# mclarsen/cuZFP

Measured on AMD Instinct MI355X. Metric: GB/s input encoded+decoded (device-resident), 3D f32 fixed-rate; % HBM peak, higher is better.
Workload: dtype f32; 1 GPU; 3d_float32_256^3_rate8; maxbits=512, parallelism=z-slab x1, stream_bytes_per_gpu=16777216

## Files before the change

cuzfp_amd/build.py:

```python
from __future__ import annotations

import os
import subprocess
import sys
from concurrent.futures import ThreadPoolExecutor

HERE = os.path.dirname(os.path.abspath(__file__))
ROOT = os.path.dirname(HERE)
CSRC = os.path.join(HERE, "csrc")
LIB = os.path.join(HERE, "lib")
BIN = os.path.join(HERE, "bin")
CLI = os.path.join(HERE, "cli")
OBJ = os.path.join(ROOT, "build", "obj")
INC = os.path.join(ROOT, "include")

ARCH = os.environ.get("CUZFP_OFFLOAD_ARCH", "gfx950")
HIPCC = os.environ.get("HIPCC", "/opt/rocm/bin/hipcc")
CXXFLAGS = ["-O3", "-std=c++17", "-fPIC", f"--offload-arch={ARCH}", f"-I{INC}",
            "-Wall", "-Wno-unused-function", "-Wno-pass-failed"]

KERNEL_UNITS = ["inst_f32", "inst_f64", "inst_i32", "inst_i64",
                "region_f32", "region_f64", "region_i32", "region_i64",
                "update_f32", "update_f64", "update_i32", "update_i64", "truncate",
                "variable_f32", "variable_f64", "region_variable_f32", "region_variable_f64", "truncate_variable",
                "region_variable_coarse_f32", "region_variable_coarse_f64",
                "region_variable_update_f32", "region_variable_update_f64",
                "capi"]
HEADERS = ["zfp_block.hpp", "kernels.hpp", "launch.hpp", "region.hpp", "region_kernels.hpp",
           "region_update_kernels.hpp", "rerate.hpp", "variable_kernels.hpp", "variable_index.hpp",
           "region_variable_kernels.hpp", "rerate_variable.hpp", "source_window.hpp", "variable_coarse.hpp",
           "region_variable_coarse_kernels.hpp", "region_variable_update_kernels.hpp"]


def _newer(target: str, deps: list[str]) -> bool:
    if not os.path.exists(target):
        return True
    t = os.path.getmtime(target)
    return any(os.path.getmtime(d) > t for d in deps)


def _run(cmd: list[str]) -> None:
    r = subprocess.run(cmd, capture_output=True, text=True)
    if r.returncode != 0:
        sys.stderr.write(r.stdout + r.stderr)
        raise RuntimeError("build failed: " + " ".join(cmd))


def build(verbose: bool = False, jobs: int | None = None) -> dict:
    os.makedirs(LIB, exist_ok=True)
    os.makedirs(OBJ, exist_ok=True)
    hdrs = [os.path.join(CSRC, h) for h in HEADERS] + [os.path.join(INC, "cuzfp_hip.h")]
    jobs_list = []
    objs = []
    for u in KERNEL_UNITS:
        src = os.path.join(CSRC, u + ".hip")
        obj = os.path.join(OBJ, u + ".o")
        objs.append(obj)
        if _newer(obj, [src] + hdrs):
            jobs_list.append([HIPCC, *CXXFLAGS, "-c", src, "-o", obj])
    with ThreadPoolExecutor(max_workers=jobs or min(8, os.cpu_count() or 4)) as ex:
        for cmd in jobs_list:
            if verbose:
                print(" ".join(cmd))
        list(ex.map(_run, jobs_list))
    hip_so = os.path.join(LIB, "libcuzfp_hip.so")
    if jobs_list or _newer(hip_so, objs):
        _run([HIPCC, f"--offload-arch={ARCH}", "-shared", "-fPIC", "-o", hip_so, *objs])
    cpp_src = os.path.join(CSRC, "cuZFP.cpp")
    cpp_so = os.path.join(LIB, "libcuZFP.so")
    if _newer(cpp_so, [cpp_src, hip_so, os.path.join(INC, "cuZFP.h"),
                       os.path.join(INC, "zfp_structs.h")]):
        _run([HIPCC, "-O2", "-std=c++17", "-fPIC", "-shared", f"-I{INC}", "-o", cpp_so, cpp_src,
              f"-L{LIB}", "-lcuzfp_hip", "-Wl,-rpath,$ORIGIN"])
    os.makedirs(BIN, exist_ok=True)
    cli = os.path.join(BIN, "cuda_zfp")
    if _newer(cli, [os.path.join(CLI, "cuda_zfp.cpp"), cpp_so, os.path.join(INC, "cuZFP.h"),
                    os.path.join(INC, "zfp_structs.h")]):
        _run(["g++", "-O2", "-std=c++17", "-Wall", "-Wno-unused-function", f"-I{INC}", "-o", cli,
              os.path.join(CLI, "cuda_zfp.cpp"), f"-L{LIB}", "-lcuZFP", "-Wl,-rpath,$ORIGIN/../lib"])
    gen = os.path.join(BIN, "data_gen")
    if _newer(gen, [os.path.join(CLI, "data_gen.cpp")]):
        _run(["g++", "-O2", "-std=c++17", "-Wall", "-o", gen, os.path.join(CLI, "data_gen.cpp")])
    return {"hip": hip_so, "cpp": cpp_so, "cli": cli, "data_gen": gen}


if __name__ == "__main__":
    print(build(verbose=True))
```

cuzfp_amd/csrc/capi.hip:

```cpp
#include <hip/hip_runtime.h>
#include <math.h>

#include <algorithm>
#include <cstring>
#include <mutex>
#include <chrono>
#include <vector>

#include "launch.hpp"
#include "rerate_variable.hpp"
#include "variable_index.hpp"

namespace cuzfp {

thread_local int t_last_hip = hipSuccess;

static unsigned min_bits(int type) { return type == CUZFP_TYPE_FLOAT ? 9 : type == CUZFP_TYPE_DOUBLE ? 12 : 1; }

static int make_problem(int type, unsigned nx, unsigned ny, unsigned nz, long long sx,
                        long long sy, long long sz, unsigned maxbits, Problem* pr) {
  if (type < CUZFP_TYPE_INT32 || type > CUZFP_TYPE_DOUBLE) return CUZFP_ERROR_UNSUPPORTED_TYPE;
  if (!nx || (nz && !ny)) return CUZFP_ERROR_INVALID_ARGUMENT;
  const unsigned dims = nz ? 3 : ny ? 2 : 1;
  const unsigned ebits = min_bits(type);
  if (maxbits < ebits || maxbits > CUZFP_MAX_BITS) return CUZFP_ERROR_INVALID_ARGUMENT;
  Geometry& g = pr->g;
  g.nx = nx;
  g.ny = dims > 1 ? ny : 1;
  g.nz = dims > 2 ? nz : 1;
  g.bx = (g.nx + 3) / 4;
  g.by = (g.ny + 3) / 4;
  const uint64_t nb = (uint64_t)g.bx * g.by * ((g.nz + 3) / 4);
  if (nb >= (1ull << 32) - kLanes) return CUZFP_ERROR_INVALID_ARGUMENT;
  g.nblocks = (uint32_t)nb;
  set_divisor(g.bx, g.dbx_m, g.dbx_s);
  set_divisor(g.bx * g.by, g.dpl_m, g.dpl_s);
  g.divmagic = nb < (1ull << 31) ? 1u : 0u;
  g.maxbits = maxbits;
  g.wave0 = 0;
  g.vec_io = 0;
  g.row_stage = 0;
  g.sx = sx ? sx : 1;
  g.sy = sy ? sy : (long long)g.nx;
  g.sz = sz ? sz : (long long)g.nx * g.ny;
  pr->type = type;
  pr->dims = dims;
  pr->fast_ok = (type == CUZFP_TYPE_FLOAT || type == CUZFP_TYPE_DOUBLE) && g.sx == 1 &&
                g.sy == (long long)g.nx && g.sz == (long long)g.nx * g.ny && g.nx % 4 == 0 &&
                (dims < 2 || g.ny % 4 == 0) && (dims < 3 || g.nz % 4 == 0);
  return CUZFP_SUCCESS;
}

static int launch_encode(const Problem& p, const void* data, uint64_t* stream, uint32_t wave0,
                         uint32_t nwaves, hipStream_t st) {
  if (!nwaves) return CUZFP_SUCCESS;
  const bool fast = p.fast_ok && ((uintptr_t)data & 15) == 0;
  switch (p.type) {
    case CUZFP_TYPE_INT32: return launch_encode_type<int32_t>(p, data, false, stream, wave0, nwaves, st);
    case CUZFP_TYPE_INT64: return launch_encode_type<int64_t>(p, data, false, stream, wave0, nwaves, st);
    case CUZFP_TYPE_FLOAT: return launch_encode_type<float>(p, data, fast, stream, wave0, nwaves, st);
    default: return launch_encode_type<double>(p, data, fast, stream, wave0, nwaves, st);
  }
}

static int launch_decode(const Problem& p, const uint64_t* stream, void* data, uint32_t wave0,
                         uint32_t nwaves, hipStream_t st) {
  if (!nwaves) return CUZFP_SUCCESS;
  const bool fast = p.fast_ok && ((uintptr_t)data & 15) == 0;
  switch (p.type) {
    case CUZFP_TYPE_INT32: return launch_decode_type<int32_t>(p, stream, false, data, wave0, nwaves, st);
    case CUZFP_TYPE_INT64: return launch_decode_type<int64_t>(p, stream, false, data, wave0, nwaves, st);
    case CUZFP_TYPE_FLOAT: return launch_decode_type<float>(p, stream, fast, data, wave0, nwaves, st);
    default: return launch_decode_type<double>(p, stream, fast, data, wave0, nwaves, st);
  }
}

static size_t stream_bytes_of(const Geometry& g) {
  return (((size_t)g.nblocks * g.maxbits + 63) / 64) * 8;
}

static uint32_t waves_of(const Geometry& g) { return (g.nblocks + kLanes - 1) / kLanes; }


typedef uint32_t u32x4 __attribute__((ext_vector_type(4)));

__global__ __launch_bounds__(256) void copy16_nt(const u32x4* __restrict__ src, u32x4* __restrict__ dst,
                                                 size_t n16) {
  const size_t stride = (size_t)gridDim.x * blockDim.x;
  for (size_t i = (size_t)blockIdx.x * blockDim.x + threadIdx.x; i < n16; i += stride)
    __builtin_nontemporal_store(__builtin_nontemporal_load(src + i), dst + i);
}


constexpr size_t kChunkBytes = 64u << 20, kStagedChunkBytes = 8u << 20;

static size_t chunk_bytes(bool staged) {
  const char* e = getenv("CUZFP_HOST_CHUNK_BYTES");
  if (e && *e) {
    const long long v = atoll(e);
    if (v > 0) return (size_t)v;
  }
  return staged ? kStagedChunkBytes : kChunkBytes;
}

static bool host_ordered() {
  const char* e = getenv("CUZFP_HOST_ORDERED");
  return !(e && *e == '0');
}

static int host_zero_copy() {
  const char* e = getenv("CUZFP_HOST_ZEROCOPY");
  return (e && *e) ? atoi(e) : 1;
}

static char* mapped_view(const void* p, size_t bytes) {
  hipPointerAttribute_t a;
  void* d = nullptr;
  hipDeviceptr_t base = nullptr;
  size_t size = 0;
  const bool ok = hipPointerGetAttributes(&a, p) == hipSuccess && a.type == hipMemoryTypeHost &&
                  hipHostGetDevicePointer(&d, const_cast<void*>(p), 0) == hipSuccess && d &&
                  hipMemGetAddressRange(&base, &size, (hipDeviceptr_t)d) == hipSuccess && base &&
                  (char*)d >= (char*)base && (size_t)((char*)d - (char*)base) + bytes <= size;
  (void)hipGetLastError();
// ... 1016 lines not shown
```

cuzfp_amd/csrc/kernels.hpp:

```cpp
#pragma once
#include <hip/hip_runtime.h>
#include <stdlib.h>

#include <atomic>
#include <type_traits>

#if defined(CUZFP_PROBE) && CUZFP_PROBE == 9
#define CUZFP_STAMP_WAVES 65536
__device__ uint64_t g_stamps[CUZFP_STAMP_WAVES * 10];
__device__ __forceinline__ uint32_t stamp_wave() { return blockIdx.x * (blockDim.x >> 6) + (threadIdx.x >> 6); }
#define ZFP_STAMP(i)                                                              \
  do {                                                                            \
    if ((threadIdx.x & 63) == 0 && stamp_wave() < CUZFP_STAMP_WAVES)              \
      g_stamps[stamp_wave() * 10 + 1 + (i)] = __builtin_amdgcn_s_memtime();      \
  } while (0)
__device__ __forceinline__ void stamp_hwid() {
  uint32_t hw, xcc;
  asm volatile("s_getreg_b32 %0, hwreg(HW_REG_HW_ID)" : "=s"(hw));
  asm volatile("s_getreg_b32 %0, hwreg(HW_REG_XCC_ID)" : "=s"(xcc));
  if ((threadIdx.x & 63) == 0 && stamp_wave() < CUZFP_STAMP_WAVES)
    g_stamps[stamp_wave() * 10] = (uint64_t)hw | ((uint64_t)xcc << 32);
}
__device__ __forceinline__ void stamp_real(int slot) {
  if ((threadIdx.x & 63) == 0 && stamp_wave() < CUZFP_STAMP_WAVES)
    g_stamps[stamp_wave() * 10 + slot] = __builtin_amdgcn_s_memrealtime();
}
#define ZFP_STAMP_REAL(slot) stamp_real(slot)
#define ZFP_STAMP_HWID() stamp_hwid()
#else
#define ZFP_STAMP_HWID()
#define ZFP_STAMP_REAL(slot)
#endif

#include "zfp_block.hpp"
#include "launch.hpp"

namespace cuzfp {

__device__ const ChunkLut g_chunk_lut = make_chunk_lut();
constexpr size_t kChunkLutBytes = sizeof(ChunkLut);
template <int DIMS>
constexpr size_t chunk_lut_bytes() { return DIMS == 1 ? kLutPairs * 4 : kChunkLutBytes; }
__device__ const SpreadTab g_spread_tab = make_spread_tab();
__device__ const Pair1dLut g_pair1d_lut = make_pair1d_lut();
__device__ const Plane1dDecLut g_plane1d_lut = make_plane1d_dec_lut();
constexpr size_t kSpreadTabBytes = sizeof(SpreadTab);
typedef __attribute__((address_space(3))) const uint32_t lds_spread;
typedef lds_spread* P1dPtr;

__device__ __forceinline__ void udivmod_uniform(uint32_t n, uint32_t d, uint32_t& q, uint32_t& r) {
  if (__builtin_expect((d & (d - 1)) == 0, 1)) {
    const uint32_t sh = (uint32_t)__builtin_ctz(d);
    q = n >> sh;
    r = n & (d - 1);
  } else {
    q = n / d;
    r = n % d;
  }
}


constexpr uint32_t kSlackWords = 6;
template <bool PRIO = true>
struct LdsOrWriter {
  static constexpr bool kPrio = PRIO;
  static constexpr bool kZeroInline = true;
  uint64_t* p;
  lds_spread* lut;
  uint32_t pos, lim;
  P1dPtr p1d;
  uint64_t fit_lim;
  __device__ __forceinline__ uint32_t pair1d(uint32_t o) const { return *(P1dPtr)((uintptr_t)p1d + o); }
  __device__ __forceinline__ bool full() const { return pos >= lim; }
  __device__ __forceinline__ void put(uint64_t v, unsigned n) {
    const uint32_t w = pos >> 6;
    uint64_t* q = p + w * 64;
    const uint64_t lo = v << (pos & 63u);
    const uint64_t hi = (v >> 1) >> ((pos ^ 63u) & 63u);
    atomicOr((unsigned long long*)&q[0], (unsigned long long)lo);
    atomicOr((unsigned long long*)&q[64], (unsigned long long)hi);
    pos += n;
  }
  __device__ __forceinline__ uint32_t sp0(uint32_t o) const { return *(lds_spread*)((uintptr_t)lut + o); }
  __device__ __forceinline__ uint32_t sp1(uint32_t o) const { return *(lds_spread*)((uintptr_t)(lut + 256) + o); }
  __device__ __forceinline__ uint32_t spread(uint32_t b) const { return lut[256 + b] >> 1; }
  __device__ __forceinline__ void zero_bit() { pos++; }
  __device__ __forceinline__ void lds_wait() const { __builtin_amdgcn_s_waitcnt(0xc07f); }
  __device__ __forceinline__ void finish() {}
  __device__ __forceinline__ void settle() { pos = pos < lim ? pos : lim; }
  __device__ __forceinline__ void mark_full(bool z) { pos = z ? lim : pos; }
};

template <bool PRIO = true>
struct LdsBitWriter {
  static constexpr bool kPrio = PRIO;
  uint64_t* lds;
  lds_spread* lut;
  uint32_t pos, end, cnt;
  uint64_t acc;
  P1dPtr p1d;
  uint64_t fit_lim;
  __device__ __forceinline__ uint32_t pair1d(uint32_t o) const { return *(P1dPtr)((uintptr_t)p1d + o); }
  __device__ __forceinline__ uint32_t sp0(uint32_t o) const { return *(lds_spread*)((uintptr_t)lut + o); }
  __device__ __forceinline__ uint32_t sp1(uint32_t o) const { return *(lds_spread*)((uintptr_t)(lut + 256) + o); }
  __device__ __forceinline__ uint32_t spread(uint32_t b) const { return lut[256 + b] >> 1; }
  __device__ __forceinline__ bool full() const { return pos + cnt >= end; }
  __device__ __forceinline__ void emit(uint64_t v) {
    if (pos >= end) return;
    const uint32_t room = end - pos;
    if (room < 64) v &= lowmask(room);
    const uint32_t w = pos >> 6, sh = pos & 63;
    atomicOr((unsigned long long*)&lds[w], (unsigned long long)(v << sh));
    if (sh) atomicOr((unsigned long long*)&lds[w + 1], (unsigned long long)(v >> (64 - sh)));
    pos += 64;
  }
  __device__ __forceinline__ void put(uint64_t v, unsigned n) {
    acc |= v << cnt;
    const unsigned c = cnt + n;
// ... 331 lines not shown
template <int DIMS>
__device__ __forceinline__ BlockPos block_pos(const Geometry& g, uint32_t b) {
  BlockPos p;
  if constexpr (DIMS == 1) {
    p.ix = b; p.iy = 0; p.iz = 0;
  } else if constexpr (DIMS == 2) {
    p.iy = g.divmagic ? div_magic(b, g.dbx_m, g.dbx_s) : b / g.bx;
    p.ix = b - p.iy * g.bx; p.iz = 0;
  } else {
    const uint32_t plane = g.bx * g.by;
    p.iz = g.divmagic ? div_magic(b, g.dpl_m, g.dpl_s) : b / plane;
    const uint32_t r = b - p.iz * plane;
    p.iy = g.divmagic ? div_magic(r, g.dbx_m, g.dbx_s) : r / g.bx;
    p.ix = r - p.iy * g.bx;
  }
  return p;
}

template <typename Scalar, int DIMS, bool FAST>
__device__ __forceinline__ void gather(const Scalar* __restrict__ data, const Geometry& g,
                                       BlockPos bp, Scalar* f) {
  constexpr int NY = DIMS > 1 ? 4 : 1, NZ = DIMS > 2 ? 4 : 1;
  if constexpr (FAST) {
    const Scalar* p = data + ((size_t)(4 * bp.iz) * g.ny + 4 * bp.iy) * g.nx + 4 * bp.ix;
#pragma unroll
    for (int z = 0; z < NZ; z++)
#pragma unroll
      for (int y = 0; y < NY; y++)
        load_row(p + ((size_t)z * g.ny + y) * g.nx, f + 16 * z + 4 * y);
  } else {
    const int wx = (int)min(4u, g.nx - 4 * bp.ix);
    const int wy = (int)min(4u, g.ny - 4 * bp.iy);
    const int wz = (int)min(4u, g.nz - 4 * bp.iz);
    const Scalar* p = data + (int64_t)(4 * bp.ix) * g.sx + (int64_t)(4 * bp.iy) * g.sy +
                      (int64_t)(4 * bp.iz) * g.sz;
#pragma unroll
    for (int z = 0; z < NZ; z++)
#pragma unroll
      for (int y = 0; y < NY; y++)
#pragma unroll
        for (int x = 0; x < 4; x++)
          f[16 * z + 4 * y + x] = p[(int64_t)pad_src(x, wx) * g.sx + (int64_t)pad_src(y, wy) * g.sy +
                                    (int64_t)pad_src(z, wz) * g.sz];
  }
}

template <typename Scalar, int DIMS, bool FAST>
__device__ __forceinline__ void scatter(Scalar* __restrict__ data, const Geometry& g, BlockPos bp,
                                        const Scalar* f) {
  constexpr int NY = DIMS > 1 ? 4 : 1, NZ = DIMS > 2 ? 4 : 1;
  if constexpr (FAST) {
    Scalar* p = data + ((size_t)(4 * bp.iz) * g.ny + 4 * bp.iy) * g.nx + 4 * bp.ix;
#pragma unroll
    for (int z = 0; z < NZ; z++)
#pragma unroll
      for (int y = 0; y < NY; y++)
        store_row(p + ((size_t)z * g.ny + y) * g.nx, f + 16 * z + 4 * y);
  } else {
    const int wx = (int)min(4u, g.nx - 4 * bp.ix);
    const int wy = (int)min(4u, g.ny - 4 * bp.iy);
    const int wz = (int)min(4u, g.nz - 4 * bp.iz);
    Scalar* p = data + (int64_t)(4 * bp.ix) * g.sx + (int64_t)(4 * bp.iy) * g.sy +
                (int64_t)(4 * bp.iz) * g.sz;
#pragma unroll
    for (int z = 0; z < NZ; z++)
#pragma unroll
      for (int y = 0; y < NY; y++)
#pragma unroll
        for (int x = 0; x < 4; x++)
          if (x < wx && y < wy && z < wz)
            p[(int64_t)x * g.sx + (int64_t)y * g.sy + (int64_t)z * g.sz] = f[16 * z + 4 * y + x];
  }
}


constexpr int kWavesPerGroup = 4;
#ifndef CUZFP_ENC_WPG
#define CUZFP_ENC_WPG 4
#endif
#ifndef CUZFP_DEC_WPG
#define CUZFP_DEC_WPG 4
#endif
constexpr int kEncWaves = CUZFP_ENC_WPG, kDecWaves = CUZFP_DEC_WPG;
#ifndef CUZFP_REG_WAVES_1D
#define CUZFP_REG_WAVES_1D 16
#endif
constexpr int kRegWaves1d = CUZFP_REG_WAVES_1D;
#ifndef CUZFP_REG_WAVES_2D
#define CUZFP_REG_WAVES_2D 4
#endif
constexpr int kRegWaves2d = CUZFP_REG_WAVES_2D;
#ifndef CUZFP_REG_DEC_BATCH_1D
#define CUZFP_REG_DEC_BATCH_1D 4
#endif
#ifndef CUZFP_REG_ENC_BATCH_1D
#define CUZFP_REG_ENC_BATCH_1D 2
#endif
#ifndef CUZFP_REG_BATCH_WAVES_1D
#define CUZFP_REG_BATCH_WAVES_1D 8
#endif
#ifndef CUZFP_REG_BATCH_MIN_WAVES
#define CUZFP_REG_BATCH_MIN_WAVES 32768
#endif
constexpr int kRegDecBatch1d = CUZFP_REG_DEC_BATCH_1D, kRegEncBatch1d = CUZFP_REG_ENC_BATCH_1D;
constexpr int kRegBatchWaves1d = CUZFP_REG_BATCH_WAVES_1D;
constexpr uint32_t kRegBatchMinWaves = CUZFP_REG_BATCH_MIN_WAVES;
#ifndef CUZFP_REG_BATCH_PRIO
#define CUZFP_REG_BATCH_PRIO 0
#endif

__device__ __forceinline__ uint32_t wave_in_group() {
  return __builtin_amdgcn_readfirstlane(threadIdx.x >> 6);
}

__device__ __forceinline__ void wave_lds_sync() {
  asm volatile("s_waitcnt lgkmcnt(0)" ::: "memory");
  __builtin_amdgcn_wave_barrier();
}

template <int ROWS>
__device__ __forceinline__ void scatter_f64_staged(double* __restrict__ data, const Geometry& g, BlockPos bp,
                                                   const double* f, bool coded, uint64_t* wave_lds,
                                                   uint32_t lane) {
  static_assert(16 % ROWS == 0, "rows a pass");
  uint4* stage = (uint4*)wave_lds;
  double* base = data + ((size_t)(4 * bp.iz) * g.ny + 4 * bp.iy) * g.nx + 4 * (bp.ix - lane);
#pragma unroll
  for (int r0 = 0; r0 < 16; r0 += ROWS) {
    if (coded) {
#pragma unroll
      for (int j = 0; j < ROWS; j++) {
        uint4 a, b;
        __builtin_memcpy(&a, f + 4 * (r0 + j), 16);
        __builtin_memcpy(&b, f + 4 * (r0 + j) + 2, 16);
        stage[j * 128 + 2 * lane] = a;
        stage[j * 128 + 2 * lane + 1] = b;
      }
    } else {
#pragma unroll
      for (int j = 0; j < ROWS; j++) {
        stage[j * 128 + 2 * lane] = uint4{0, 0, 0, 0};
        stage[j * 128 + 2 * lane + 1] = uint4{0, 0, 0, 0};
      }
    }
    wave_lds_sync();
#pragma unroll
    for (int j = 0; j < ROWS; j++) {
      const int r = r0 + j, z = r >> 2, y = r & 3;
      double* row = base + ((size_t)z * g.ny + y) * g.nx;
      st16<true>(row + 2 * lane, stage[j * 128 + lane]);
      st16<true>(row + 128 + 2 * lane, stage[j * 128 + 64 + lane]);
    }
    if (r0 + ROWS < 16) wave_lds_sync();
  }
}

#ifndef CUZFP_F64_ENC_WAVES
#define CUZFP_F64_ENC_WAVES 2
#endif
#ifndef CUZFP_F64_DEC_WAVES
#define CUZFP_F64_DEC_WAVES 2
#endif
#ifndef CUZFP_F32_DEC_WAVES
#define CUZFP_F32_DEC_WAVES 4
#endif
#ifndef CUZFP_F32_ENC_WAVES
// ... 82 lines not shown
    if (g.wave0 + (bid + 1) * (blockDim.x >> 6) <= g.wave_end) {
      asm volatile("s_waitcnt vmcnt(0)" ::: "memory");
      __syncthreads();
    }
    wave_lds_sync();
    LdsOrWriter<PRIO> wr{mine, lut, 0, 64 * W, p1d, uniform_const64(0x7fffu)};
    encode_block<Scalar, DIMS>(f, g.maxbits, wr);
  } else if (b < g.nblocks) {
    {
      wave_lds_sync();
      LdsBitWriter<PRIO> wr{lds, lut, lane * g.maxbits, (lane + 1) * g.maxbits, 0, 0, p1d, uniform_const64(0x7fffu)};
      encode_block<Scalar, DIMS>(f, g.maxbits, wr);
    }
  }
  if constexpr (PRIO) __builtin_amdgcn_s_setprio(3);
  wave_lds_sync();
  const uint32_t nb = min((uint32_t)kLanes, g.nblocks - wave * kLanes);
  const uint32_t nwords = (nb * g.maxbits + 63) >> 6;
  uint64_t* out = stream + (size_t)wave * g.maxbits;
  if constexpr (ALIGNED) {
    if (nb == kLanes && g.vec_io && !(W & 1)) {
      uint32_t s, j, ds, dj;
      udivmod_uniform(2 * lane, W, s, j);
      udivmod_uniform(128u, W, ds, dj);
      for (uint32_t k = 2 * lane; k < kLanes * W; k += 128) {
        uint4 v;
        const uint64_t a0 = lds[j * 64 + s], a1 = lds[(j + 1) * 64 + s];
        __builtin_memcpy(&v.x, &a0, 8);
        __builtin_memcpy(&v.z, &a1, 8);
        st16<true>(&out[k], v);
        j += dj;
        s += ds;
        if (j >= W) { j -= W; s++; }
      }
      ZFP_STAMP(6);
      ZFP_STAMP_REAL(9);
      return;
    }
  }
  if constexpr (ALIGNED) {
    if (b < g.nblocks) {
      const uint64_t* mine = lds + lane;
      uint64_t* dst = out + (size_t)lane * W;
      if (g.vec_io && !(W & 1)) {
        for (uint32_t j = 0; j < W; j += 2) {
          uint4 v;
          const uint64_t a0 = mine[j * 64], a1 = mine[(j + 1) * 64];
          __builtin_memcpy(&v.x, &a0, 8);
          __builtin_memcpy(&v.z, &a1, 8);
          st16<kNtStream>(&dst[j], v);
        }
      } else {
        for (uint32_t j = 0; j < W; j++) dst[j] = mine[j * 64];
      }
    }
  } else if (g.vec_io) {
    const uint32_t npairs = nwords >> 1;
    for (uint32_t j = lane; j < npairs; j += kLanes)
      ((uint4*)out)[j] = ((const uint4*)lds)[j];
    if ((nwords & 1) && lane == 0) out[nwords - 1] = lds[nwords - 1];
  } else {
    for (uint32_t j = lane; j < nwords; j += kLanes) out[j] = lds[j];
  }
  ZFP_STAMP(6);
  ZFP_STAMP_REAL(9);
}

template <typename Scalar, int DIMS, bool FAST, bool ALIGNED, bool PRIO = true, int REG = 0, int WPG = kEncWaves>
__global__ __launch_bounds__(kLanes * WPG, (occupancy<Scalar, DIMS, true>::value)) void zfp_encode(const Scalar* __restrict__ data,
                                                                      Geometry g,
                                                                      uint64_t* __restrict__ stream) {
  __shared__ __attribute__((aligned(16))) uint32_t stab[512];
  __shared__ __attribute__((aligned(16))) uint32_t ptab[DIMS == 1 ? 1024 : 4];
  zfp_encode_body<Scalar, DIMS, FAST, ALIGNED, PRIO, REG, WPG>(data, g, stream, blockIdx.x, stab, ptab);
}

template <typename Scalar, int DIMS, bool FAST, bool PRIO = true, int REG = 0, int WPG = kDecWaves>
__device__ __forceinline__ void zfp_decode_body(const uint64_t* __restrict__ stream, const Geometry& g,
                                                Scalar* __restrict__ data, uint32_t bid,
                                                uint32_t* ctab, uint16_t* dtab) {
  extern __shared__ __attribute__((aligned(16))) uint64_t lds_all[];
  constexpr int N = 1 << (2 * DIMS);
  const uint32_t wig = wave_in_group();
  const uint32_t wave = g.wave0 + bid * (blockDim.x >> 6) + wig;
  const uint32_t lane = threadIdx.x & 63;
  const uint32_t b = wave * kLanes + lane;
  const bool live = wave < g.wave_end && b < g.nblocks;
  uint64_t* lds = lds_all + (size_t)wig * g.lds_words;
  uint32_t* lut = ctab;
  auto copy_dtab = [&]() {
    if constexpr (DIMS == 1)
      for (uint32_t i = threadIdx.x; i < sizeof(Plane1dDecLut) / 16; i += blockDim.x)
        ((uint4*)dtab)[i] = ((const uint4*)g_plane1d_lut.e)[i];
  };
  constexpr uint32_t kLutEnd = DIMS == 1 ? kLutPairs * 4 / 16 : sizeof(ChunkLut) / 16;
  const uint32_t* seg = (const uint32_t*)(stream + (size_t)wave * g.maxbits);
  uint32_t* L = (uint32_t*)lds + lane;
  uint64_t blk = 0;
  if constexpr (REG == 32) {
    if (live) blk = seg[lane];
    for (uint32_t i = threadIdx.x; i < kLutEnd; i += blockDim.x)
      ((uint4*)lut)[i] = ((const uint4*)g_chunk_lut.e)[i];
    copy_dtab();
  } else if constexpr (REG) {
    if (live) {
      const uint32_t nb = min((uint32_t)kLanes, g.nblocks - wave * kLanes);
      const uint32_t lim = ((nb * g.maxbits + 63) >> 6) * 2;
      const uint32_t s0 = lane * g.maxbits, d0 = s0 >> 5;
      const uint32_t a0 = seg[d0];
      const uint32_t a1 = d0 + 1 < lim ? seg[d0 + 1] : 0u;
      const uint32_t a2 = d0 + 2 < lim ? seg[d0 + 2] : 0u;
      blk = ((uint64_t)__builtin_amdgcn_alignbit(a1, a0, s0) |
             ((uint64_t)__builtin_amdgcn_alignbit(a2, a1, s0) << 32)) & lowmask(g.maxbits);
    }
    for (uint32_t i = threadIdx.x; i < kLutEnd; i += blockDim.x)
      ((uint4*)lut)[i] = ((const uint4*)g_chunk_lut.e)[i];
    copy_dtab();
  } else {
    const uint32_t D = (g.maxbits + 31) >> 5;
    const bool vec = (g.maxbits & 127) == 0 && g.vec_io;
    constexpr uint32_t kHeld = 8;
    uint4 held[kHeld];
    const bool cont = vec && wave < g.wave_end && g.nblocks - wave * kLanes >= kLanes && D <= 4 * kHeld;
    if (cont) {
      const uint4* src = (const uint4*)seg + lane;
#pragma unroll
      for (uint32_t q = 0; q < kHeld; q++)
        if (4 * q < D) held[q] = ld16<true>(&src[64 * q]);
    } else if (live && vec) {
      const uint4* src = (const uint4*)(seg + lane * D);
#pragma unroll
      for (uint32_t q = 0; q < kHeld; q++)
        if (4 * q < D) held[q] = ld16<kNtStream>(&src[q]);
    }
    for (uint32_t i = threadIdx.x; i < kLutEnd; i += blockDim.x)
      ((uint4*)lut)[i] = ((const uint4*)g_chunk_lut.e)[i];
    copy_dtab();
    if (cont) {
      uint32_t* L0 = (uint32_t*)lds;
      uint32_t sb, j, dsb, dj;
      udivmod_uniform(4 * lane, D, sb, j);
      udivmod_uniform(256u, D, dsb, dj);
#pragma unroll
      for (uint32_t q = 0; q < kHeld; q++)
        if (4 * q < D) {
          L0[(j) * 64 + sb] = held[q].x;
          L0[(j + 1) * 64 + sb] = held[q].y;
          L0[(j + 2) * 64 + sb] = held[q].z;
          L0[(j + 3) * 64 + sb] = held[q].w;
          j += dj;
          sb += dsb;
          if (j >= D) { j -= D; sb++; }
        }
    } else if (live) {
      if (vec) {
#pragma unroll
        for (uint32_t q = 0; q < kHeld; q++)
          if (4 * q < D) {
            L[(4 * q) * 64] = held[q].x;
            L[(4 * q + 1) * 64] = held[q].y;
            L[(4 * q + 2) * 64] = held[q].z;
            L[(4 * q + 3) * 64] = held[q].w;
          }
        const uint4* src = (const uint4*)(seg + lane * D);
        for (uint32_t q = 4 * kHeld; q < D; q += 4) {
          const uint4 v = src[q >> 2];
          L[q * 64] = v.x;
// ... 145 lines not shown
  a2 = d0 + 2 < lim ? a2 : 0u;
  return ((uint64_t)__builtin_amdgcn_alignbit(a1, a0, s0) | ((uint64_t)__builtin_amdgcn_alignbit(a2, a1, s0) << 32)) &
         lowmask(g.maxbits);
}

template <typename Scalar, int DIMS, bool FAST, bool PRIO, int WPG, int K, int REG = 64>
__global__ __launch_bounds__(kLanes * WPG, (occupancy<Scalar, DIMS>::value)) void zfp_decode_regk(
    const uint64_t* __restrict__ stream, Geometry g, Scalar* __restrict__ data) {
  static_assert(DIMS <= 2 && K >= 2 && K <= 8, "register-reader batches: 1D/2D, 2-8 a wave");
  constexpr int N = 1 << (2 * DIMS);
  __shared__ __attribute__((aligned(16))) uint32_t ctab[chunk_lut_bytes<DIMS>() / 4];
  __shared__ __attribute__((aligned(16))) uint16_t dtab[DIMS == 1 ? sizeof(Plane1dDecLut) / 2 : 8];
  const uint32_t wig = wave_in_group();
  const uint32_t lane = threadIdx.x & 63;
  const uint32_t w0 = g.wave0 + (blockIdx.x * WPG + wig) * K;
  uint64_t q[K];
#pragma unroll
  for (int k = 0; k < K; k++) {
    const uint32_t w = w0 + k;
    if (w < g.wave_end && w * kLanes + lane < g.nblocks)
      q[k] = REG == 32 ? (uint64_t)((const uint32_t*)(stream + (size_t)w * g.maxbits))[lane] : reg_block(stream, g, w, lane);
    else
      q[k] = 0;
  }
  constexpr uint32_t kLutEnd = DIMS == 1 ? kLutPairs * 4 / 16 : sizeof(ChunkLut) / 16;
  for (uint32_t i = threadIdx.x; i < kLutEnd; i += blockDim.x) ((uint4*)ctab)[i] = ((const uint4*)g_chunk_lut.e)[i];
  if constexpr (DIMS == 1)
    for (uint32_t i = threadIdx.x; i < sizeof(Plane1dDecLut) / 16; i += blockDim.x)
      ((uint4*)dtab)[i] = ((const uint4*)g_plane1d_lut.e)[i];
  __syncthreads();
  const uint32_t nw = w0 < g.wave_end ? min((uint32_t)K, g.wave_end - w0) : 0u;
#pragma unroll 1
  for (uint32_t k = 0; k < nw; k++) {
    const uint64_t blk = q[0];
#pragma unroll
    for (int j = 0; j + 1 < K; j++) q[j] = q[j + 1];
    const uint32_t b = (w0 + k) * kLanes + lane;
    if constexpr (PRIO) __builtin_amdgcn_s_setprio(3);
    Scalar f[N];
    RegReader<PRIO, REG == 32> rd;
    rd.lds32 = nullptr;
    rd.lut32 = ctab;
    rd.d1d = dtab;
    rd.set_block(blk);
    rd.init(0);
    const bool coded = decode_block<Scalar, DIMS>(f, g.maxbits, rd);
    if constexpr (PRIO) __builtin_amdgcn_s_setprio(3);
    if (!coded) {
#pragma unroll
      for (int i = 0; i < N; i++) f[i] = (Scalar)0;
    }
    if (b < g.nblocks) scatter<Scalar, DIMS, FAST>(data, g, block_pos<DIMS>(g, b), f);
  }
}


static inline size_t lds_cap_bytes() {
  static const long forced = [] {
    const char* e = getenv("CUZFP_LDS_CAP_BYTES");
    return (e && *e) ? atol(e) : 0L;
  }();
  if (forced > 0) return (size_t)forced;
  static std::atomic<int> cap[kMaxDevices];
  int dev = 0;
  if (hipGetDevice(&dev) != hipSuccess || dev < 0 || dev >= kMaxDevices) return 65536;
  int c = cap[dev].load(std::memory_order_relaxed);
  if (!c) {
    int n = 0;
    if (hipDeviceGetAttribute(&n, hipDeviceAttributeMaxSharedMemoryPerBlock, dev) != hipSuccess || n <= 0)
      n = 65536;
    cap[dev].store(n, std::memory_order_relaxed);
    c = n;
  }
  return (size_t)c;
}

static inline uint32_t waves_per_group(uint32_t lds_words, size_t shared_bytes, uint32_t most) {
  const size_t cap = lds_cap_bytes();
  uint32_t w = most;
  while (w > 1 && (size_t)w * lds_words * 8 + shared_bytes > cap) w >>= 1;
  return w;
}

static inline bool use_priority(uint32_t nwaves, int waves_per_simd, uint32_t rounds) {
  static const int forced = [] {
    const char* e = getenv("CUZFP_PRIO");
    return (e && *e) ? (atoi(e) != 0 ? 1 : 0) : -1;
  }();
  if (forced >= 0) return forced != 0;
  static std::atomic<int> cus[kMaxDevices];
  int dev = 0, c = 256;
  if (hipGetDevice(&dev) == hipSuccess && dev >= 0 && dev < kMaxDevices) {
    c = cus[dev].load(std::memory_order_relaxed);
    if (!c) {
      int n = 0;
      if (hipDeviceGetAttribute(&n, hipDeviceAttributeMultiprocessorCount, dev) != hipSuccess || n <= 0) n = 256;
      cus[dev].store(n, std::memory_order_relaxed);
      c = n;
    }
  }
  return nwaves <= (uint32_t)c * 4u * (uint32_t)waves_per_simd * rounds;
}

#if defined(CUZFP_XVAR)
constexpr bool kFastOnly = true;
#else
constexpr bool kFastOnly = false;
#endif
#ifndef CUZFP_ENC_PRIO_ROUNDS
#define CUZFP_ENC_PRIO_ROUNDS 1
#endif
template <typename Scalar, int DIMS>
int launch_encode_t(const void* data, const Geometry& g, bool fast, uint64_t* stream,
                           uint32_t wave0, uint32_t nwaves, hipStream_t st) {
  Geometry gg = g;
  gg.wave0 = wave0;
  gg.wave_end = wave0 + nwaves;
  gg.vec_io = (g.maxbits % 2 == 0) && ((uintptr_t)stream % 16 == 0);
  gg.lds_words = g.maxbits + kLanes * kSlackWords;
  constexpr size_t kStatic = kSpreadTabBytes + (DIMS == 1 ? sizeof(Pair1dLut) : 16);
  const Scalar* d = (const Scalar*)data;
  if constexpr (DIMS <= 2) {
    if (g.maxbits == 32 || g.maxbits == 64) {
      gg.lds_words = 0;
      const dim3 grid((nwaves + kWavesPerGroup - 1) / kWavesPerGroup), block(kLanes * kWavesPerGroup);
      const bool prio = use_priority(nwaves, occupancy<Scalar, DIMS, true>::value, CUZFP_ENC_PRIO_ROUNDS);
#define ZFP_ENC_REG(FAST_, PRIO_)                                                                          \
  do {                                                                                                     \
    if (g.maxbits == 64)                                                                                   \
      hipLaunchKernelGGL((zfp_encode<Scalar, DIMS, FAST_, true, PRIO_, 2, kWavesPerGroup>), grid, block, 0, st, d, gg, stream); \
    else                                                                                                   \
      hipLaunchKernelGGL((zfp_encode<Scalar, DIMS, FAST_, true, PRIO_, 1, kWavesPerGroup>), grid, block, 0, st, d, gg, stream); \
  } while (0)
      if constexpr (DIMS == 1 && kRegEncBatch1d > 1) {
        if (fast && nwaves >= kRegBatchMinWaves) {
          constexpr int W = kWavesPerGroup, K = kRegEncBatch1d;
          const uint32_t phys = (nwaves + K - 1) / K;
          const dim3 kgrid((phys + W - 1) / W), kblock(kLanes * W);
          if (g.maxbits == 64)
            hipLaunchKernelGGL((zfp_encode_regk<Scalar, DIMS, false, 2, W, K>), kgrid, kblock, 0, st, d, gg, stream);
          else
            hipLaunchKernelGGL((zfp_encode_regk<Scalar, DIMS, false, 1, W, K>), kgrid, kblock, 0, st, d, gg, stream);
          const hipError_t e = hipGetLastError();
          t_last_hip = e;
          return e == hipSuccess ? CUZFP_SUCCESS : CUZFP_ERROR_HIP;
        }
      }
      if (fast && prio) ZFP_ENC_REG(true, true);
      else if (fast) ZFP_ENC_REG(true, false);
      else if (prio) ZFP_ENC_REG(false, true);
      else ZFP_ENC_REG(false, false);
#undef ZFP_ENC_REG
      const hipError_t e = hipGetLastError();
      t_last_hip = e;
      return e == hipSuccess ? CUZFP_SUCCESS : CUZFP_ERROR_HIP;
    }
  }
  const bool aligned = (g.maxbits & 63) == 0 && gg.lds_words * 8 + kStatic <= lds_cap_bytes();
  if (!aligned) gg.lds_words = g.maxbits + 2;
  gg.row_stage = 0;
  if (gg.lds_words * 8 + kStatic > lds_cap_bytes()) return CUZFP_ERROR_INVALID_ARGUMENT;
  const uint32_t wpg = waves_per_group(gg.lds_words, kStatic, kEncWaves);
  const dim3 grid((nwaves + wpg - 1) / wpg), block(kLanes * wpg);
  const size_t lds = (size_t)wpg * gg.lds_words * 8;
  if (fast && aligned && !use_priority(nwaves, occupancy<Scalar, DIMS, true>::value, CUZFP_ENC_PRIO_ROUNDS))
    hipLaunchKernelGGL((zfp_encode<Scalar, DIMS, true, true, false>), grid, block, lds, st, d, gg, stream);
  else if (fast && aligned)
    hipLaunchKernelGGL((zfp_encode<Scalar, DIMS, true, true>), grid, block, lds, st, d, gg, stream);
  else if (fast)
    hipLaunchKernelGGL((zfp_encode<Scalar, DIMS, true, false>), grid, block, lds, st, d, gg, stream);
  else if constexpr (kFastOnly)
    return CUZFP_ERROR_UNSUPPORTED_TYPE;
  else if (aligned)
    hipLaunchKernelGGL((zfp_encode<Scalar, DIMS, false, true>), grid, block, lds, st, d, gg, stream);
  else
    hipLaunchKernelGGL((zfp_encode<Scalar, DIMS, false, false>), grid, block, lds, st, d, gg, stream);
  const hipError_t e = hipGetLastError();
  t_last_hip = e;
  return e == hipSuccess ? CUZFP_SUCCESS : CUZFP_ERROR_HIP;
}

template <typename Scalar, int DIMS>
int launch_decode_t(const uint64_t* stream, const Geometry& g, bool fast, void* data,
                           uint32_t wave0, uint32_t nwaves, hipStream_t st) {
  Geometry gg = g;
  gg.wave0 = wave0;
  gg.wave_end = wave0 + nwaves;
  gg.vec_io = (g.maxbits % 2 == 0) && ((uintptr_t)stream % 16 == 0);
  gg.lds_words = ((g.maxbits + 31) / 32 + 5) * 32;
  gg.row_stage = 0;
  if (sizeof(Scalar) == 8 && DIMS == 3 && fast && g.bx % kLanes == 0) {
    const size_t img = (size_t)gg.lds_words * 8;
    gg.row_stage = img >= 4 * 2048 ? 4 : img >= 2 * 2048 ? 2 : img >= 2048 ? 1 : 0;
  }
  const bool reg = DIMS <= 2 && g.maxbits <= 64;
  if (reg) gg.lds_words = 0;
  const size_t kStatic = chunk_lut_bytes<DIMS>() + (DIMS == 1 ? sizeof(Plane1dDecLut) : 16);
  if (gg.lds_words * 8 + kStatic > lds_cap_bytes()) return CUZFP_ERROR_INVALID_ARGUMENT;
  const uint32_t wpg = waves_per_group(gg.lds_words, kStatic, kDecWaves);
  const dim3 grid((nwaves + wpg - 1) / wpg), block(kLanes * wpg);
  const size_t lds = (size_t)wpg * gg.lds_words * 8;
  Scalar* d = (Scalar*)data;
  if constexpr (DIMS <= 2) {
    if (reg) {
      const bool prio = use_priority(nwaves, occupancy<Scalar, DIMS>::value, 2);
      if constexpr (DIMS == 1 && kRegDecBatch1d > 1) {
        if (fast && nwaves >= kRegBatchMinWaves) {
          constexpr int W = kRegBatchWaves1d, K = kRegDecBatch1d;
          const uint32_t phys = (nwaves + K - 1) / K;
          const dim3 kgrid((phys + W - 1) / W), kblock(kLanes * W);
          constexpr bool P = CUZFP_REG_BATCH_PRIO;
          if (g.maxbits == 32)
            hipLaunchKernelGGL((zfp_decode_regk<Scalar, DIMS, true, P, W, K, 32>), kgrid, kblock, 0, st, stream, gg, d);
          else
            hipLaunchKernelGGL((zfp_decode_regk<Scalar, DIMS, true, P, W, K, 64>), kgrid, kblock, 0, st, stream, gg, d);
          const hipError_t e = hipGetLastError();
          t_last_hip = e;
          return e == hipSuccess ? CUZFP_SUCCESS : CUZFP_ERROR_HIP;
        }
      }
      constexpr int W = DIMS == 1 ? kRegWaves1d : kRegWaves2d;
      const dim3 rgrid((nwaves + W - 1) / W), rblock(kLanes * W);
      auto go = [&](auto rb) {
        constexpr int RB = decltype(rb)::value;
        if (fast && prio)
          hipLaunchKernelGGL((zfp_decode<Scalar, DIMS, true, true, RB, W>), rgrid, rblock, 0, st, stream, gg, d);
        else if (fast)
          hipLaunchKernelGGL((zfp_decode<Scalar, DIMS, true, false, RB, W>), rgrid, rblock, 0, st, stream, gg, d);
        else if (prio)
          hipLaunchKernelGGL((zfp_decode<Scalar, DIMS, false, true, RB, W>), rgrid, rblock, 0, st, stream, gg, d);
        else
          hipLaunchKernelGGL((zfp_decode<Scalar, DIMS, false, false, RB, W>), rgrid, rblock, 0, st, stream, gg, d);
      };
      if (g.maxbits == 32)
        go(std::integral_constant<int, 32>{});
      else
        go(std::integral_constant<int, 64>{});
      const hipError_t e = hipGetLastError();
      t_last_hip = e;
      return e == hipSuccess ? CUZFP_SUCCESS : CUZFP_ERROR_HIP;
    }
  }
  constexpr uint32_t kDecPrioRounds = (sizeof(Scalar) == 8 && DIMS == 3) ? 1 : 2;
  if (fast && !use_priority(nwaves, occupancy<Scalar, DIMS>::value, kDecPrioRounds))
    hipLaunchKernelGGL((zfp_decode<Scalar, DIMS, true, false>), grid, block, lds, st, stream, gg, d);
  else if (fast)
    hipLaunchKernelGGL((zfp_decode<Scalar, DIMS, true>), grid, block, lds, st, stream, gg, d);
  else if constexpr (!kFastOnly)
    hipLaunchKernelGGL((zfp_decode<Scalar, DIMS, false>), grid, block, lds, st, stream, gg, d);
  const hipError_t e = hipGetLastError();
  t_last_hip = e;
  return e == hipSuccess ? CUZFP_SUCCESS : CUZFP_ERROR_HIP;
}


#if defined(CUZFP_XVAR)
#include "../../tools/xvar_launch.hpp"
#else
template <typename Scalar>
int launch_encode_type(const Problem& p, const void* data, bool fast, uint64_t* stream,
                       uint32_t wave0, uint32_t nwaves, hipStream_t st) {
  switch (p.dims) {
    case 1: return launch_encode_t<Scalar, 1>(data, p.g, fast, stream, wave0, nwaves, st);
    case 2: return launch_encode_t<Scalar, 2>(data, p.g, fast, stream, wave0, nwaves, st);
    default: return launch_encode_t<Scalar, 3>(data, p.g, fast, stream, wave0, nwaves, st);
  }
}

template <typename Scalar>
int launch_decode_type(const Problem& p, const uint64_t* stream, bool fast, void* data,
                       uint32_t wave0, uint32_t nwaves, hipStream_t st) {
  switch (p.dims) {
    case 1: return launch_decode_t<Scalar, 1>(stream, p.g, fast, data, wave0, nwaves, st);
    case 2: return launch_decode_t<Scalar, 2>(stream, p.g, fast, data, wave0, nwaves, st);
    default: return launch_decode_t<Scalar, 3>(stream, p.g, fast, data, wave0, nwaves, st);
  }
}

#endif

}
```

cuzfp_amd/csrc/launch.hpp:

```cpp
#pragma once
#include <hip/hip_runtime.h>
#include <stdint.h>

#include "../../include/cuzfp_hip.h"
#include "region.hpp"

namespace cuzfp {

constexpr int kLanes = 64;
constexpr int kMaxDevices = 64;

struct Geometry {
  uint32_t nx, ny, nz;
  uint32_t bx, by;
  uint32_t nblocks;
  uint32_t maxbits;
  uint32_t wave0;
  uint32_t wave_end;
  uint32_t vec_io;
  uint32_t lds_words;
  int64_t sx, sy, sz;
  uint32_t dbx_m, dbx_s, dpl_m, dpl_s, divmagic;
  uint32_t row_stage;
};

inline void set_divisor(uint32_t d, uint32_t& m, uint32_t& s) {
  uint32_t l = 0;
  while ((1ull << l) < d) l++;
  s = 31 + l;
  m = (uint32_t)(((1ull << s) + d - 1) / d);
}

inline Region make_region(const Geometry& g, uint32_t ox, uint32_t oy, uint32_t oz, uint32_t ex,
                          uint32_t ey, uint32_t ez, int64_t sx, int64_t sy, int64_t sz) {
  Region r;
  r.bx = g.bx;
  r.by = g.by;
  r.bx0 = ox / 4;
  r.by0 = oy / 4;
  r.bz0 = oz / 4;
  r.rbx = (uint32_t)(((uint64_t)ox + ex + 3) / 4) - r.bx0;
  r.rby = (uint32_t)(((uint64_t)oy + ey + 3) / 4) - r.by0;
  r.rbz = (uint32_t)(((uint64_t)oz + ez + 3) / 4) - r.bz0;
  const uint64_t n = (uint64_t)r.rbx * r.rby * r.rbz;
  r.nrb = (uint32_t)n;
  r.ox = ox; r.oy = oy; r.oz = oz;
  r.ex = ex; r.ey = ey; r.ez = ez;
  r.maxbits = g.maxbits;
  set_divisor(r.rbx, r.drx_m, r.drx_s);
  set_divisor(r.rbx * r.rby, r.drp_m, r.drp_s);
  r.divmagic = n < (1ull << 31) ? 1u : 0u;
  r.stream_dwords = (((uint64_t)g.nblocks * g.maxbits + 63) / 64) * 2;
  r.sx = sx ? sx : 1;
  r.sy = sy ? sy : (int64_t)ex;
  r.sz = sz ? sz : (int64_t)ex * ey;
  return r;
}

struct Problem {
  int type;
  unsigned dims;
  Geometry g;
  bool fast_ok;
};

extern thread_local int t_last_hip;

template <typename Scalar>
int launch_encode_type(const Problem& p, const void* data, bool fast, uint64_t* stream,
                       uint32_t wave0, uint32_t nwaves, hipStream_t st);
template <typename Scalar>
int launch_decode_type(const Problem& p, const uint64_t* stream, bool fast, void* data,
                       uint32_t wave0, uint32_t nwaves, hipStream_t st);
template <typename Scalar>
int launch_decode_region_type(const Problem& p, const Region& r, const uint64_t* stream, bool fast,
                              uint32_t budget, void* out, hipStream_t st);

inline bool region_covered(const Geometry& g, const Region& r) {
  auto axis = [](uint32_t o, uint32_t e, uint32_t n) { return !(o & 3) && (!((o + e) & 3) || o + e == n); };
  return axis(r.ox, r.ex, g.nx) && axis(r.oy, r.ey, g.ny) && axis(r.oz, r.ez, g.nz);
}

template <typename Scalar>
int launch_encode_region_type(const Problem& p, const Region& r, const void* box, bool covered, bool rows,
                              uint64_t* stream, hipStream_t st);

int launch_truncate(const uint64_t* src, uint64_t* dst, uint32_t nblocks, uint32_t M, uint32_t m, hipStream_t st);

constexpr uint32_t kVariableScanTile = 1024;
inline uint32_t variable_tiles(uint32_t nblocks) { return (nblocks + kVariableScanTile - 1) / kVariableScanTile; }
int launch_variable_scan(const uint16_t* lengths, uint32_t nblocks, uint64_t* offsets, uint64_t* partials,
                         uint64_t* total, hipStream_t st);
int launch_variable_zero(uint64_t* stream, uint64_t cap_words, const uint64_t* offsets, uint32_t nblocks,
                         const uint64_t* total, hipStream_t st);
template <typename Scalar>
int launch_encode_variable_type(const Problem& p, const void* data, bool fast, uint32_t maxprec, int minexp,
                                uint64_t* stream, uint64_t cap_words, uint16_t* lengths, uint64_t* total,
                                uint64_t* offsets, uint64_t* partials, hipStream_t st);
template <typename Scalar>
int launch_decode_variable_type(const Problem& p, const uint64_t* stream, size_t stream_bytes,
                                const uint16_t* lengths, bool fast, void* out, uint64_t* offsets,
                                uint64_t* partials, hipStream_t st);

int launch_truncate_variable(bool is_double, unsigned dims, const uint64_t* src, size_t src_bytes,
                             const uint16_t* src_lengths, uint32_t nblocks, uint32_t new_maxprec, int new_minexp,
                             uint64_t* dst, uint64_t cap_words, uint16_t* lengths, uint64_t* total,
// ... 23 lines not shown
```

Before: 1435 GB/s.

## Launch 3D f32 decode with larger workgroups and XCD-aware wave remapping

For 3D float decode, adds a path that launches workgroups of 16 waves instead of the default and remaps each group's waves so that each XCD decodes the same wave indices the encoder's smaller groups placed there. The aim is to keep each XCD's decode reading stream data that its own L2/MALL slice likely still holds from the encode, and to cut per-group launch overhead. The path is gated on divisibility, LDS capacity and priority conditions, and it assumes round-robin dispatch of workgroups across 8 XCDs. Larger groups may lower occupancy, or fall back when the conditions fail.

```diff
diff --git a/cuzfp_amd/build.py b/cuzfp_amd/build.py
--- a/cuzfp_amd/build.py
+++ b/cuzfp_amd/build.py
@@ -26,7 +26,7 @@
                 "region_variable_coarse_f32", "region_variable_coarse_f64",
                 "region_variable_update_f32", "region_variable_update_f64",
                 "capi"]
-HEADERS = ["zfp_block.hpp", "kernels.hpp", "launch.hpp", "region.hpp", "region_kernels.hpp",
+HEADERS = ["zfp_block.hpp", "kernels.hpp", "launch.hpp", "wave_index.hpp", "region.hpp", "region_kernels.hpp",
            "region_update_kernels.hpp", "rerate.hpp", "variable_kernels.hpp", "variable_index.hpp",
            "region_variable_kernels.hpp", "rerate_variable.hpp", "source_window.hpp", "variable_coarse.hpp",
            "region_variable_coarse_kernels.hpp", "region_variable_update_kernels.hpp"]
diff --git a/cuzfp_amd/csrc/capi.hip b/cuzfp_amd/csrc/capi.hip
--- a/cuzfp_amd/csrc/capi.hip
+++ b/cuzfp_amd/csrc/capi.hip
@@ -40,6 +40,7 @@
   g.wave0 = 0;
   g.vec_io = 0;
   g.row_stage = 0;
+  g.xcd_remap = 0;
   g.sx = sx ? sx : 1;
   g.sy = sy ? sy : (long long)g.nx;
   g.sz = sz ? sz : (long long)g.nx * g.ny;
diff --git a/cuzfp_amd/csrc/kernels.hpp b/cuzfp_amd/csrc/kernels.hpp
--- a/cuzfp_amd/csrc/kernels.hpp
+++ b/cuzfp_amd/csrc/kernels.hpp
@@ -34,6 +34,7 @@
 
 #include "zfp_block.hpp"
 #include "launch.hpp"
+#include "wave_index.hpp"
 
 namespace cuzfp {
 
@@ -531,6 +532,10 @@
 #define CUZFP_DEC_WPG 4
 #endif
 constexpr int kEncWaves = CUZFP_ENC_WPG, kDecWaves = CUZFP_DEC_WPG;
+#ifndef CUZFP_DEC_WPG_ROUND
+#define CUZFP_DEC_WPG_ROUND 16
+#endif
+constexpr int kDecWavesRound = CUZFP_DEC_WPG_ROUND;
 #ifndef CUZFP_REG_WAVES_1D
 #define CUZFP_REG_WAVES_1D 16
 #endif
@@ -779,7 +784,11 @@
   extern __shared__ __attribute__((aligned(16))) uint64_t lds_all[];
   constexpr int N = 1 << (2 * DIMS);
   const uint32_t wig = wave_in_group();
-  const uint32_t wave = g.wave0 + bid * (blockDim.x >> 6) + wig;
+  uint32_t wave;
+  if constexpr (DIMS == 3 && !REG)
+    wave = g.wave0 + decode_wave_of(bid, wig, blockDim.x >> 6, kEncWaves, g.xcd_remap != 0);
+  else
+    wave = g.wave0 + bid * (blockDim.x >> 6) + wig;
   const uint32_t lane = threadIdx.x & 63;
   const uint32_t b = wave * kLanes + lane;
   const bool live = wave < g.wave_end && b < g.nblocks;
@@ -1091,12 +1100,7 @@
   return w;
 }
 
-static inline bool use_priority(uint32_t nwaves, int waves_per_simd, uint32_t rounds) {
-  static const int forced = [] {
-    const char* e = getenv("CUZFP_PRIO");
-    return (e && *e) ? (atoi(e) != 0 ? 1 : 0) : -1;
-  }();
-  if (forced >= 0) return forced != 0;
+static inline bool within_rounds(uint32_t nwaves, int waves_per_simd, uint32_t rounds) {
   static std::atomic<int> cus[kMaxDevices];
   int dev = 0, c = 256;
   if (hipGetDevice(&dev) == hipSuccess && dev >= 0 && dev < kMaxDevices) {
@@ -1109,6 +1113,14 @@
     }
   }
   return nwaves <= (uint32_t)c * 4u * (uint32_t)waves_per_simd * rounds;
+}
+static inline bool use_priority(uint32_t nwaves, int waves_per_simd, uint32_t rounds) {
+  static const int forced = [] {
+    const char* e = getenv("CUZFP_PRIO");
+    return (e && *e) ? (atoi(e) != 0 ? 1 : 0) : -1;
+  }();
+  if (forced >= 0) return forced != 0;
+  return within_rounds(nwaves, waves_per_simd, rounds);
 }
 
 #if defined(CUZFP_XVAR)
@@ -1251,6 +1263,26 @@
     }
   }
   constexpr uint32_t kDecPrioRounds = (sizeof(Scalar) == 8 && DIMS == 3) ? 1 : 2;
+  if constexpr (DIMS == 3 && sizeof(Scalar) == 4 && kDecWavesRound > kDecWaves) {
+    constexpr uint32_t R = kDecWavesRound;
+    if (within_rounds(nwaves, occupancy<Scalar, DIMS>::value, 1) && decode_remap_ok(nwaves, R, kEncWaves) &&
+        (size_t)R * gg.lds_words * 8 + kStatic <= lds_cap_bytes() &&
+        waves_per_group(g.maxbits + kLanes * kSlackWords, kSpreadTabBytes + 16, kEncWaves) == (uint32_t)kEncWaves &&
+        use_priority(nwaves, occupancy<Scalar, DIMS>::value, kDecPrioRounds)) {
+      gg.xcd_remap = 1;
+      const dim3 rgrid(nwaves / R), rblock(kLanes * R);
+      const size_t rlds = (size_t)R * gg.lds_words * 8;
+      if (fast)
+        hipLaunchKernelGGL((zfp_decode<Scalar, DIMS, true, true, 0, R>), rgrid, rblock, rlds, st, stream, gg, d);
+      else if constexpr (!kFastOnly)
+        hipLaunchKernelGGL((zfp_decode<Scalar, DIMS, false, true, 0, R>), rgrid, rblock, rlds, st, stream, gg, d);
+      else
+        return CUZFP_ERROR_UNSUPPORTED_TYPE;
+      const hipError_t e = hipGetLastError();
+      t_last_hip = e;
+      return e == hipSuccess ? CUZFP_SUCCESS : CUZFP_ERROR_HIP;
+    }
+  }
   if (fast && !use_priority(nwaves, occupancy<Scalar, DIMS>::value, kDecPrioRounds))
     hipLaunchKernelGGL((zfp_decode<Scalar, DIMS, true, false>), grid, block, lds, st, stream, gg, d);
   else if (fast)
diff --git a/cuzfp_amd/csrc/launch.hpp b/cuzfp_amd/csrc/launch.hpp
--- a/cuzfp_amd/csrc/launch.hpp
+++ b/cuzfp_amd/csrc/launch.hpp
@@ -22,6 +22,7 @@
   int64_t sx, sy, sz;
   uint32_t dbx_m, dbx_s, dpl_m, dpl_s, divmagic;
   uint32_t row_stage;
+  uint32_t xcd_remap;
 };
 
 inline void set_divisor(uint32_t d, uint32_t& m, uint32_t& s) {
diff --git a/cuzfp_amd/csrc/wave_index.hpp b/cuzfp_amd/csrc/wave_index.hpp
--- /dev/null
+++ b/cuzfp_amd/csrc/wave_index.hpp
@@ -0,0 +1,25 @@
+#pragma once
+#include <stdint.h>
+
+#if defined(__HIPCC__)
+#define CUZFP_WI_HD __host__ __device__ __forceinline__
+#else
+#define CUZFP_WI_HD inline
+#endif
+
+namespace cuzfp {
+
+constexpr uint32_t kXcds = 8;
+
+CUZFP_WI_HD bool decode_remap_ok(uint32_t nwaves, uint32_t wpg, uint32_t enc_wpg) {
+  return enc_wpg != 0 && wpg > enc_wpg && wpg % enc_wpg == 0 && nwaves % (kXcds * wpg) == 0;
+}
+
+CUZFP_WI_HD uint32_t decode_wave_of(uint32_t group, uint32_t wig, uint32_t wpg, uint32_t enc_wpg, bool remap) {
+  if (!remap) return group * wpg + wig;
+  const uint32_t x = group % kXcds, q = group / kXcds;
+  const uint32_t t = wig / enc_wpg, w = wig % enc_wpg;
+  return enc_wpg * (kXcds * ((wpg / enc_wpg) * q + t) + x) + w;
+}
+
+}
```

New measurement: 1450 GB/s, median of 6. 1.01x the previous value.
